# kmaninis/OSVOS-PyTorch

Hardware: NVIDIA H100
Metric: frames/sec at 480x854 fwd-only, batch 1 per GPU (OSVOS.forward -> 5 logit maps) (higher is better)
Workload: dtype bf16x3 (split-bf16 operands, fp32 accumulate)

## Files before the change

### osvos_pytorch_b200/csrc/conv_common.cuh

```cuda
#pragma once
#include <stdlib.h>

#include "common.cuh"
#include "ptx.cuh"

namespace osvos {

constexpr int kTileW = 8;
constexpr int kTileH = 16;
constexpr int kBlockM = 128;
constexpr int kBlockK = 64;
constexpr int kConvThreads = 384;
constexpr int kABytes = kBlockM * kBlockK * 2;

struct ConvParams {
  const float* bias;
  __nv_bfloat16* y_hi;
  __nv_bfloat16* y_lo;
  float* y_f32;
  const __nv_bfloat16* mask_hi;
  __nv_bfloat16* pool_hi;
  __nv_bfloat16* pool_lo;
  float* colsum;
  int n, h, w, cin, cout;
  int tiles_x, tiles_y, n_blocks, total_tiles, k_chunks;
  int flags;
  int ablate;
};

__device__ __forceinline__ void decode_tile(const ConvParams& p, int tile, int& nb, int& tx, int& ty, int& img) {
  nb = tile % p.n_blocks;
  int m = tile / p.n_blocks;
  tx = m % p.tiles_x;
  m /= p.tiles_x;
  ty = m % p.tiles_y;
  img = m / p.tiles_y;
}

__device__ __forceinline__ uint32_t sw128_offset(int row, int chunk) { return row * 128 + ((chunk ^ (row & 7)) << 4); }

__device__ __forceinline__ void split_pack2(float a, float b, uint32_t& hi, uint32_t& lo) {
  asm("cvt.rn.bf16x2.f32 %0, %1, %2;" : "=r"(hi) : "f"(b), "f"(a));
  const float ra = a - __uint_as_float(hi << 16);
  const float rb = b - __uint_as_float(hi & 0xFFFF0000u);
  asm("cvt.rn.bf16x2.f32 %0, %1, %2;" : "=r"(lo) : "f"(rb), "f"(ra));
}

template <int BLOCK_N, bool SPLIT_ACC, bool LEAN = false, bool DET = false>
__device__ __forceinline__ void conv_epilogue(const ConvParams& p, const float* acc, int tile, int wg, int wl, int lane) {
  if (p.ablate & 16) return;
  int nb, tx, ty, img;
  decode_tile(p, tile, nb, tx, ty, img);
  const int lx = lane >> 2;
  const int x = tx * kTileW + lx;
  const int y0 = ty * kTileH + wg * 8 + wl * 2;
  const bool va = (y0 < p.h) && (x < p.w), vb = (y0 + 1 < p.h) && (x < p.w);
  const bool relu = (p.flags & OSVOS_FLAG_RELU) != 0;
  const bool masked = !LEAN && (p.flags & OSVOS_FLAG_RELU_MASK) != 0;
  const bool store_ok = !(p.ablate & 8);
  const size_t pix[2] = {(static_cast<size_t>(img) * p.h + y0) * p.w + x, (static_cast<size_t>(img) * p.h + y0 + 1) * p.w + x};
  const bool valid[2] = {va, vb};
  const int oh = (p.h + 1) >> 1, ow = (p.w + 1) >> 1;
  const bool pool_writer = va && !(lx & 1) && store_ok;
  const size_t opix = (static_cast<size_t>(img) * oh + (y0 >> 1)) * ow + (x >> 1);
#pragma unroll
  for (int j = 0; j < BLOCK_N / 8; ++j) {
    const int c = 8 * j + 2 * (lane & 3);
    const int ch = nb * BLOCK_N + c;
    const float2 b = p.bias ? __ldg(reinterpret_cast<const float2*>(p.bias + ch)) : make_float2(0.f, 0.f);
    float f[2][2];
#pragma unroll
    for (int h = 0; h < 2; ++h) {
#pragma unroll
      for (int e = 0; e < 2; ++e) {
        float v = e ? b.y : b.x;
        v += acc[4 * j + 2 * h + e];
        if (SPLIT_ACC) v += acc[BLOCK_N / 2 + 4 * j + 2 * h + e];
        f[h][e] = relu ? fmaxf(v, 0.f) : v;
      }
    }
#pragma unroll
    for (int h = 0; h < 2; ++h) {
      if (!LEAN && masked && valid[h]) {
        const uint32_t m = __ldg(reinterpret_cast<const unsigned int*>(p.mask_hi + pix[h] * p.cout + ch));
        if (!(bf16_lo_to_float(m) > 0.f)) f[h][0] = 0.f;
        if (!(bf16_hi_to_float(m) > 0.f)) f[h][1] = 0.f;
      }
      if (valid[h] && store_ok) {
        if (!LEAN && p.y_f32) *reinterpret_cast<float2*>(p.y_f32 + pix[h] * p.cout + ch) = make_float2(f[h][0], f[h][1]);
        if (p.y_hi) {
          uint32_t hi, lo;
          split_pack2(f[h][0], f[h][1], hi, lo);
          *reinterpret_cast<uint32_t*>(p.y_hi + pix[h] * p.cout + ch) = hi;
          if (p.y_lo) *reinterpret_cast<uint32_t*>(p.y_lo + pix[h] * p.cout + ch) = lo;
        }
      }
    }
    if (!LEAN && p.colsum) {
      float s0 = (va ? f[0][0] : 0.f) + (vb ? f[1][0] : 0.f);
      float s1 = (va ? f[0][1] : 0.f) + (vb ? f[1][1] : 0.f);
#pragma unroll
      for (int o = 4; o <= 16; o <<= 1) {
        s0 += __shfl_xor_sync(0xffffffffu, s0, o);
        s1 += __shfl_xor_sync(0xffffffffu, s1, o);
      }
      if (lane < 4) {
        if constexpr (DET) {
          const size_t prow = (static_cast<size_t>(tile / p.n_blocks) * 2 + wg) * 4 + wl;
          *reinterpret_cast<float2*>(p.colsum + prow * p.cout + ch) = make_float2(s0, s1);
        } else {
          atomicAdd(p.colsum + ch, s0);
          atomicAdd(p.colsum + ch + 1, s1);
        }
      }
    }
    if (p.pool_hi) {
      float m0 = fmaxf(va ? f[0][0] : -INFINITY, vb ? f[1][0] : -INFINITY);
      float m1 = fmaxf(va ? f[0][1] : -INFINITY, vb ? f[1][1] : -INFINITY);
      m0 = fmaxf(m0, __shfl_xor_sync(0xffffffffu, m0, 4));
      m1 = fmaxf(m1, __shfl_xor_sync(0xffffffffu, m1, 4));
      if (pool_writer) {
        uint32_t hi, lo;
        split_pack2(m0, m1, hi, lo);
        *reinterpret_cast<uint32_t*>(p.pool_hi + opix * p.cout + ch) = hi;
        if (p.pool_lo) *reinterpret_cast<uint32_t*>(p.pool_lo + opix * p.cout + ch) = lo;
      }
    }
  }
}

constexpr int kStageBoxBytes = 64 * 64 * 2;

struct OutMaps {
  CUtensorMap y_hi, y_lo;
};

__device__ __forceinline__ void conv_epilogue_staged(const ConvParams& p, const OutMaps& maps, const float* acc, int tile,
                                                     int half, int wl, int lane, uint8_t* box, int bar_id, bool leader) {
  if (p.ablate & 16) return;
  int nb, tx, ty, img;
  decode_tile(p, tile, nb, tx, ty, img);
  const int lx = lane >> 2;
  const bool relu = (p.flags & OSVOS_FLAG_RELU) != 0;
  const bool store_ok = !(p.ablate & 8);
  const int planes = p.y_lo ? 2 : 1;
  const uint32_t act_row = smem_u32(box) + (wl * 2 * 8 + lx) * 128;
  const uint32_t col = 4 * (lane & 3);
#pragma unroll 1
  for (int plane = 0; plane < planes; ++plane) {
    if (leader) bulk_wait_group_read<0>();
    named_bar_sync(bar_id, 128);
#pragma unroll
    for (int j = 0; j < 8; ++j) {
      const int ch = nb * 64 + 8 * j + 2 * (lane & 3);
      const float2 b = p.bias ? __ldg(reinterpret_cast<const float2*>(p.bias + ch)) : make_float2(0.f, 0.f);
      float f[2][2];
#pragma unroll
      for (int h = 0; h < 2; ++h) {
#pragma unroll
        for (int e = 0; e < 2; ++e) {
          float v = e ? b.y : b.x;
          v += acc[4 * j + 2 * h + e];
          f[h][e] = relu ? fmaxf(v, 0.f) : v;
        }
      }
#pragma unroll
      for (int h = 0; h < 2; ++h) {
        uint32_t hi, lo;
        split_pack2(f[h][0], f[h][1], hi, lo);
        st_shared_u32(act_row + h * 8 * 128 + ((j ^ lx) << 4) + col, plane ? lo : hi);
      }
    }
    fence_proxy_async_smem();
    named_bar_sync(bar_id, 128);
    if (leader && store_ok) {
      tma_store_4d(plane ? &maps.y_lo : &maps.y_hi, box, nb * 64, tx * kTileW, ty * kTileH + half * 8, img);
      bulk_commit_group();
    }
  }
}


static inline void fill_conv_params(ConvParams& p, const osvos_conv3x3_args* a, int block_n) {
  p.bias = a->bias;
  p.y_hi = static_cast<__nv_bfloat16*>(a->y_hi);
  p.y_lo = static_cast<__nv_bfloat16*>(a->y_lo);
  p.y_f32 = a->y_f32;
  p.mask_hi = static_cast<const __nv_bfloat16*>(a->mask_hi);
  p.pool_hi = static_cast<__nv_bfloat16*>(a->pool_hi);
  p.pool_lo = static_cast<__nv_bfloat16*>(a->pool_lo);
  p.colsum = a->colsum;
  p.n = a->n;
  p.h = a->h;
  p.w = a->w;
  p.cin = a->cin;
  p.cout = a->cout;
  p.tiles_x = (a->w + kTileW - 1) / kTileW;
  p.tiles_y = (a->h + kTileH - 1) / kTileH;
  p.n_blocks = a->cout / block_n;
  p.total_tiles = p.tiles_x * p.tiles_y * a->n * p.n_blocks;
  p.k_chunks = a->cin / kBlockK;
  p.flags = a->flags;
  {
    static int ablate = -1;
    if (ablate < 0) {
      const char* e = getenv("OSVOS_ABLATE");
      ablate = e ? atoi(e) : 0;
    }
    p.ablate = ablate;
  }
}

static inline int encode_weight_maps(CUtensorMap* hi, CUtensorMap* lo, const osvos_conv3x3_args* a, int block_n) {
  const size_t plane = static_cast<size_t>(9) * a->cout * a->cin;
  const uint64_t dims[3] = {(uint64_t)a->cin, (uint64_t)a->cout, 9};
  const uint64_t strides[2] = {(uint64_t)a->cin * 2, (uint64_t)a->cout * a->cin * 2};
  const uint32_t box[3] = {kBlockK, (uint32_t)block_n, 1};
  const __nv_bfloat16* wp = static_cast<const __nv_bfloat16*>(a->w_packed);
  int rc = encode_tensor_map(hi, CU_TENSOR_MAP_DATA_TYPE_BFLOAT16, 2, 3, wp, dims, strides, box,
                             CU_TENSOR_MAP_SWIZZLE_128B);
  if (rc) return rc;
  return encode_tensor_map(lo, CU_TENSOR_MAP_DATA_TYPE_BFLOAT16, 2, 3, wp + plane, dims, strides, box,
                           CU_TENSOR_MAP_SWIZZLE_128B);
}

static inline bool outputs_tma_aligned(const osvos_conv3x3_args* a) {
  return ((reinterpret_cast<uintptr_t>(a->y_hi) | reinterpret_cast<uintptr_t>(a->y_lo)) & 15) == 0;
}

static inline int encode_output_maps(OutMaps* m, const osvos_conv3x3_args* a) {
  memset(m, 0, sizeof(*m));
  const uint64_t c = a->cout;
  const uint64_t dims[4] = {c, (uint64_t)a->w, (uint64_t)a->h, (uint64_t)a->n};
  const uint64_t strides[3] = {c * 2, c * 2 * a->w, c * 2 * a->w * a->h};
  const uint32_t box[4] = {64, kTileW, kTileH / 2, 1};
  int rc = encode_tensor_map(&m->y_hi, CU_TENSOR_MAP_DATA_TYPE_BFLOAT16, 2, 4, a->y_hi, dims, strides, box,
                             CU_TENSOR_MAP_SWIZZLE_128B);
  if (rc == OSVOS_OK && a->y_lo)
    rc = encode_tensor_map(&m->y_lo, CU_TENSOR_MAP_DATA_TYPE_BFLOAT16, 2, 4, a->y_lo, dims, strides, box,
                           CU_TENSOR_MAP_SWIZZLE_128B);
  return rc;
}

int conv_first_tc_launch(const float* x, const float* w_oihw, const float* bias, void* y_hi, void* y_lo, int n, int h,
                         int w, int flags, cudaStream_t stream);
int side_conv_dispatch(const osvos_conv3x3_args* a, cudaStream_t stream);
int side_conv_multi_dispatch(const osvos_conv3x3_args* const* args, int count, cudaStream_t stream);

}
```

### osvos_pytorch_b200/csrc/conv_first_tc.cu

```cuda
#include <string.h>

#include "conv_common.cuh"

namespace osvos {

constexpr int kFirstStages = 3;
constexpr int kFirstStageBytes = 2 * kABytes;
constexpr int kFirstBBytes = 2 * 64 * 128;
template <bool STAGED>
constexpr int kFirstSmem = kFirstStages * kFirstStageBytes + kFirstBBytes + (STAGED ? 2 * kStageBoxBytes : 0) + 1024 + 256;

template <int PLANES, bool STAGED>
__global__ void __launch_bounds__(kConvThreads, 1)
conv_first_tc_kernel(const float* __restrict__ x, const float* __restrict__ wgt, const __grid_constant__ OutMaps out,
                     const ConvParams p) {
  extern __shared__ uint8_t smem_raw[];
  uint8_t* smem = reinterpret_cast<uint8_t*>((reinterpret_cast<uintptr_t>(smem_raw) + 1023) & ~uintptr_t(1023));
  uint8_t* smem_b = smem + kFirstStages * kFirstStageBytes;
  uint8_t* smem_stage = smem_b + kFirstBBytes;
  uint64_t* bars = reinterpret_cast<uint64_t*>(smem_stage + (STAGED ? 2 * kStageBoxBytes : 0));
  uint64_t* full_bar = bars;
  uint64_t* empty_bar = bars + kFirstStages;

  const int warp = threadIdx.x >> 5;
  const int lane = threadIdx.x & 31;

  if (threadIdx.x == 0) {
    for (int i = 0; i < kFirstStages; ++i) {
      mbar_init(&full_bar[i], 128);
      mbar_init(&empty_bar[i], 2);
    }
    fence_barrier_init();
  }
  pdl_wait();
  pdl_launch_dependents();
  for (int i = threadIdx.x; i < 64 * 4; i += kConvThreads) {
    const int co = i >> 2, chunk = i & 3;
    uint32_t hi[4], lo[4];
#pragma unroll
    for (int t = 0; t < 4; ++t) {
      const int k0 = chunk * 8 + 2 * t;
      const float v0 = k0 < 27 ? wgt[co * 27 + k0] : 0.f;
      const float v1 = k0 + 1 < 27 ? wgt[co * 27 + k0 + 1] : 0.f;
      __nv_bfloat16 h0, l0, h1, l1;
      split_bf16(v0, h0, l0);
      split_bf16(v1, h1, l1);
      hi[t] = pack_bf16x2(h0, h1);
      lo[t] = pack_bf16x2(l0, l1);
    }
    *reinterpret_cast<uint4*>(smem_b + sw128_offset(co, chunk)) = make_uint4(hi[0], hi[1], hi[2], hi[3]);
    *reinterpret_cast<uint4*>(smem_b + 64 * 128 + sw128_offset(co, chunk)) = make_uint4(lo[0], lo[1], lo[2], lo[3]);
  }
  fence_proxy_async_smem();
  __syncthreads();

  if (warp >= 4) {
    const int wg = (warp - 4) >> 2, wl = warp & 3;
    const bool leader = (threadIdx.x & 127) == 0;
    const uint64_t db_hi = make_smem_desc(smem_b, 16, 1024, kDescSW128);
    const uint64_t db_lo = db_hi + ((64 * 128) >> 4);
    int stage = 0;
    uint32_t phase = 0;
    float acc[32];
    for (int tile = blockIdx.x; tile < p.total_tiles; tile += gridDim.x) {
      mbar_wait(&full_bar[stage], phase);
      const uint64_t da_hi = make_smem_desc(smem + stage * kFirstStageBytes + wg * 64 * 128, 16, 1024, kDescSW128);
      const uint64_t da_lo = da_hi + (kABytes >> 4);
#pragma unroll
      for (int i = 0; i < 32; ++i) acc[i] = 0.f;
      wgmma_fence();
#pragma unroll
      for (int k = 0; k < 2; ++k) {
        if (PLANES == 2) {
          wgmma_bf16<64>(acc, da_lo + 2 * k, db_hi + 2 * k, 1);
          wgmma_bf16<64>(acc, da_hi + 2 * k, db_lo + 2 * k, 1);
        }
        wgmma_bf16<64>(acc, da_hi + 2 * k, db_hi + 2 * k, 1);
      }
      wgmma_commit();
      wgmma_wait<0>();
      wgmma_fence_operands(acc);
      if (leader) mbar_arrive(&empty_bar[stage]);
      if (++stage == kFirstStages) {
        stage = 0;
        phase ^= 1;
      }
      if constexpr (STAGED)
        conv_epilogue_staged(p, out, acc, tile, wg, wl, lane, smem_stage + wg * kStageBoxBytes, 1 + wg, leader);
      else
        conv_epilogue<64, false>(p, acc, tile, wg, wl, lane);
    }
    if (STAGED && leader) bulk_wait_group<0>();
  } else {
    const int row = threadIdx.x;
    const int ly = row / kTileW, lx = row % kTileW;
    int stage = 0;
    uint32_t phase = 0;
    const size_t plane_sz = static_cast<size_t>(p.h) * p.w;
    auto load_tile = [&](int tile, float (&v)[27]) {
      int nb, tx, ty, img;
      decode_tile(p, tile, nb, tx, ty, img);
      const int y = ty * kTileH + ly, xx = tx * kTileW + lx;
#pragma unroll
      for (int ci = 0; ci < 3; ++ci) {
        const float* pl = x + (static_cast<size_t>(img) * 3 + ci) * plane_sz;
#pragma unroll
        for (int r = 0; r < 3; ++r) {
          const int iy = y + r - 1;
#pragma unroll
          for (int s = 0; s < 3; ++s) {
            const int ix = xx + s - 1;
            v[ci * 9 + r * 3 + s] =
                (iy >= 0 && iy < p.h && ix >= 0 && ix < p.w) ? __ldg(pl + static_cast<size_t>(iy) * p.w + ix) : 0.f;
          }
        }
      }
    };
    float vn[27];
    if (static_cast<int>(blockIdx.x) < p.total_tiles) load_tile(blockIdx.x, vn);
    for (int tile = blockIdx.x; tile < p.total_tiles; tile += gridDim.x) {
      float v[32];
#pragma unroll
      for (int k = 0; k < 27; ++k) v[k] = vn[k];
#pragma unroll
      for (int k = 27; k < 32; ++k) v[k] = 0.f;
      if (tile + static_cast<int>(gridDim.x) < p.total_tiles) load_tile(tile + gridDim.x, vn);
      mbar_wait(&empty_bar[stage], phase ^ 1);
      uint8_t* st = smem + stage * kFirstStageBytes;
#pragma unroll
      for (int chunk = 0; chunk < 4; ++chunk) {
        uint32_t hi[4], lo[4];
#pragma unroll
        for (int t = 0; t < 4; ++t) {
          __nv_bfloat16 h0, l0, h1, l1;
          split_bf16(v[chunk * 8 + 2 * t], h0, l0);
          split_bf16(v[chunk * 8 + 2 * t + 1], h1, l1);
          hi[t] = pack_bf16x2(h0, h1);
          lo[t] = pack_bf16x2(l0, l1);
        }
        *reinterpret_cast<uint4*>(st + sw128_offset(row, chunk)) = make_uint4(hi[0], hi[1], hi[2], hi[3]);
        if (PLANES == 2)
          *reinterpret_cast<uint4*>(st + kABytes + sw128_offset(row, chunk)) = make_uint4(lo[0], lo[1], lo[2], lo[3]);
      }
      fence_proxy_async_smem();
      mbar_arrive(&full_bar[stage]);
      if (++stage == kFirstStages) {
        stage = 0;
        phase ^= 1;
      }
    }
  }
}

int conv_first_tc_launch(const float* x, const float* w_oihw, const float* bias, void* y_hi, void* y_lo, int n, int h,
                         int w, int flags, cudaStream_t stream) {
  osvos_conv3x3_args a;
  memset(&a, 0, sizeof(a));
  a.bias = bias;
  a.y_hi = y_hi;
  a.y_lo = (flags & OSVOS_FLAG_FAST) ? nullptr : y_lo;
  a.n = n;
  a.h = h;
  a.w = w;
  a.cin = 64;
  a.cout = 64;
  a.flags = flags;
  ConvParams p;
  fill_conv_params(p, &a, 64);
  const bool fast = (flags & OSVOS_FLAG_FAST) != 0;
  const bool staged = outputs_tma_aligned(&a);
  OutMaps out;
  if (staged) {
    const int rc = encode_output_maps(&out, &a);
    if (rc) return rc;
  } else {
    memset(&out, 0, sizeof(out));
  }
  auto kern = staged ? (fast ? conv_first_tc_kernel<1, true> : conv_first_tc_kernel<2, true>)
                     : (fast ? conv_first_tc_kernel<1, false> : conv_first_tc_kernel<2, false>);
  const int smem = staged ? kFirstSmem<true> : kFirstSmem<false>;
  static uint64_t attr_done[4] = {0, 0, 0, 0};
  OSVOS_CHECK_CUDA(ensure_dynamic_smem(kern, smem, &attr_done[(staged ? 2 : 0) + (fast ? 1 : 0)]));
  const int sms = device_sm_count();
  const int grid = p.total_tiles < sms ? p.total_tiles : sms;
  OSVOS_CHECK_CUDA(launch_pdl(kern, dim3(grid), dim3(kConvThreads), smem, stream, x, w_oihw, out, p));
  return OSVOS_OK;
}

}
```

### osvos_pytorch_b200/csrc/ptx.cuh

```cuda
#pragma once
#include <cuda.h>
#include <cuda_runtime.h>
#include <stdint.h>

#include "wgmma.cuh"

namespace osvos {

#ifndef OSVOS_SPIN_LIMIT
#define OSVOS_SPIN_LIMIT (1u << 26)
#endif

__device__ __forceinline__ uint32_t smem_u32(const void* p) {
  return static_cast<uint32_t>(__cvta_generic_to_shared(p));
}

__device__ __forceinline__ bool elect_one() {
  uint32_t pred = 0;
  asm volatile(
      "{\n\t.reg .pred P;\n\t"
      "elect.sync _|P, 0xffffffff;\n\t"
      "selp.u32 %0, 1, 0, P;\n\t}\n"
      : "=r"(pred));
  return pred != 0;
}

__device__ __forceinline__ void pdl_wait() { asm volatile("griddepcontrol.wait;" ::: "memory"); }
__device__ __forceinline__ void pdl_launch_dependents() { asm volatile("griddepcontrol.launch_dependents;" ::: "memory"); }

__device__ __forceinline__ void mbar_init(uint64_t* bar, uint32_t count) {
  asm volatile("mbarrier.init.shared::cta.b64 [%0], %1;" ::"r"(smem_u32(bar)), "r"(count) : "memory");
}
__device__ __forceinline__ void fence_barrier_init() {
  asm volatile("fence.mbarrier_init.release.cluster;" ::: "memory");
}
__device__ __forceinline__ void fence_proxy_async_smem() {
  asm volatile("fence.proxy.async.shared::cta;" ::: "memory");
}
__device__ __forceinline__ void mbar_arrive_expect_tx(uint64_t* bar, uint32_t bytes) {
  asm volatile("mbarrier.arrive.expect_tx.shared::cta.b64 _, [%0], %1;" ::"r"(smem_u32(bar)), "r"(bytes)
               : "memory");
}
__device__ __forceinline__ void mbar_arrive(uint64_t* bar) {
  asm volatile("mbarrier.arrive.shared::cta.b64 _, [%0];" ::"r"(smem_u32(bar)) : "memory");
}
__device__ __forceinline__ bool mbar_try_wait(uint64_t* bar, uint32_t parity) {
  uint32_t ok;
  asm volatile(
      "{\n\t.reg .pred P;\n\t"
      "mbarrier.try_wait.parity.shared::cta.b64 P, [%1], %2;\n\t"
      "selp.u32 %0, 1, 0, P;\n\t}\n"
      : "=r"(ok)
      : "r"(smem_u32(bar)), "r"(parity)
      : "memory");
  return ok != 0;
}

__device__ __forceinline__ void mbar_wait(uint64_t* bar, uint32_t parity) {
  uint32_t spins = 0;
  while (!mbar_try_wait(bar, parity)) {
    if (++spins > OSVOS_SPIN_LIMIT) __trap();
  }
}

__device__ __forceinline__ void cp_async_8_zfill(void* dst, const void* src, uint32_t src_bytes) {
  asm volatile("cp.async.ca.shared.global [%0], [%1], 8, %2;" ::"r"(smem_u32(dst)), "l"(src), "r"(src_bytes) : "memory");
}
__device__ __forceinline__ void cp_async_mbar_arrive_noinc(uint64_t* bar) {
  asm volatile("cp.async.mbarrier.arrive.noinc.shared::cta.b64 [%0];" ::"r"(smem_u32(bar)) : "memory");
}

__device__ __forceinline__ void tma_prefetch_desc(const CUtensorMap* m) {
  asm volatile("prefetch.tensormap [%0];" ::"l"(reinterpret_cast<uint64_t>(m)) : "memory");
}
__device__ __forceinline__ void tma_load_4d(const CUtensorMap* m, uint64_t* bar, void* dst, int c0, int c1, int c2,
                                            int c3) {
  asm volatile(
      "cp.async.bulk.tensor.4d.shared::cluster.global.mbarrier::complete_tx::bytes"
      " [%0], [%1, {%3, %4, %5, %6}], [%2];"
      ::"r"(smem_u32(dst)), "l"(reinterpret_cast<uint64_t>(m)), "r"(smem_u32(bar)), "r"(c0), "r"(c1), "r"(c2),
      "r"(c3)
      : "memory");
}
__device__ __forceinline__ void tma_load_2d(const CUtensorMap* m, uint64_t* bar, void* dst, int c0, int c1) {
  asm volatile(
      "cp.async.bulk.tensor.2d.shared::cluster.global.mbarrier::complete_tx::bytes"
      " [%0], [%1, {%3, %4}], [%2];"
      ::"r"(smem_u32(dst)), "l"(reinterpret_cast<uint64_t>(m)), "r"(smem_u32(bar)), "r"(c0), "r"(c1)
      : "memory");
}
__device__ __forceinline__ void tma_load_3d(const CUtensorMap* m, uint64_t* bar, void* dst, int c0, int c1, int c2) {
  asm volatile(
      "cp.async.bulk.tensor.3d.shared::cluster.global.mbarrier::complete_tx::bytes"
      " [%0], [%1, {%3, %4, %5}], [%2];"
      ::"r"(smem_u32(dst)), "l"(reinterpret_cast<uint64_t>(m)), "r"(smem_u32(bar)), "r"(c0), "r"(c1), "r"(c2)
      : "memory");
}
__device__ __forceinline__ void st_shared_u32(uint32_t addr, uint32_t v) {
  asm volatile("st.shared.u32 [%0], %1;" ::"r"(addr), "r"(v) : "memory");
}
__device__ __forceinline__ void tma_store_4d(const CUtensorMap* m, const void* src, int c0, int c1, int c2, int c3) {
  asm volatile(
      "cp.async.bulk.tensor.4d.global.shared::cta.bulk_group [%0, {%2, %3, %4, %5}], [%1];"
      ::"l"(reinterpret_cast<uint64_t>(m)), "r"(smem_u32(src)), "r"(c0), "r"(c1), "r"(c2), "r"(c3)
      : "memory");
}
__device__ __forceinline__ void bulk_commit_group() { asm volatile("cp.async.bulk.commit_group;" ::: "memory"); }
template <int N>
__device__ __forceinline__ void bulk_wait_group_read() { asm volatile("cp.async.bulk.wait_group.read %0;" ::"n"(N) : "memory"); }
template <int N>
__device__ __forceinline__ void bulk_wait_group() { asm volatile("cp.async.bulk.wait_group %0;" ::"n"(N) : "memory"); }

constexpr uint64_t kDescSW128 = 1ull << 62;
__host__ __device__ constexpr uint64_t desc_template(uint32_t lbo_bytes, uint32_t sbo_bytes, uint64_t layout) {
  return (static_cast<uint64_t>((lbo_bytes >> 4) & 0x3FFF) << 16) | (static_cast<uint64_t>((sbo_bytes >> 4) & 0x3FFF) << 32) |
         layout;
}
__device__ __forceinline__ uint64_t make_smem_desc(const void* p, uint32_t lbo_bytes, uint32_t sbo_bytes, uint64_t layout) {
  return desc_template(lbo_bytes, sbo_bytes, layout) | static_cast<uint64_t>((smem_u32(p) >> 4) & 0x3FFF);
}

__device__ __forceinline__ void named_bar_sync(int id, int nthreads) {
  asm volatile("bar.sync %0, %1;" ::"r"(id), "r"(nthreads) : "memory");
}
__device__ __forceinline__ void named_bar_arrive(int id, int nthreads) {
  asm volatile("bar.arrive %0, %1;" ::"r"(id), "r"(nthreads) : "memory");
}

template <int N>
__device__ __forceinline__ void setmaxnreg_dec() { asm volatile("setmaxnreg.dec.sync.aligned.u32 %0;" ::"n"(N)); }
template <int N>
__device__ __forceinline__ void setmaxnreg_inc() { asm volatile("setmaxnreg.inc.sync.aligned.u32 %0;" ::"n"(N)); }

struct StageRelease {
  uint64_t* bar_b = nullptr;
  uint64_t* bar_a = nullptr;
  __device__ __forceinline__ void release(bool leader) {
    if (leader) {
      if (bar_b) mbar_arrive(bar_b);
      if (bar_a) mbar_arrive(bar_a);
    }
    bar_b = bar_a = nullptr;
  }
};

}
```

Measured before the change: 659.1.

## Pipeline first-conv input patches via cp.async and per-warp staged TMA epilogue stores

The first-layer producer now loads each tile's 3x18x10 input halo patch into shared memory with a 4-slot cp.async ring, instead of each thread doing 27 guarded global loads with a register prefetch. The staged epilogue is changed from two 128-thread named-barrier rounds per plane to per-warp double-buffered boxes of two rows. These boxes write hi and lo together and issue the TMA stores from lane 0, and each warp waits only for an older slot. This targets global-load latency and epilogue synchronisation, at the cost of more shared memory and smaller TMA store boxes. The output tensor map box changes to 2 rows, which affects every user of encode_output_maps.

```diff
diff --git a/osvos_pytorch_b200/csrc/conv_common.cuh b/osvos_pytorch_b200/csrc/conv_common.cuh
--- a/osvos_pytorch_b200/csrc/conv_common.cuh
+++ b/osvos_pytorch_b200/csrc/conv_common.cuh
@@ -129,54 +129,61 @@
   }
 }
 
-constexpr int kStageBoxBytes = 64 * 64 * 2;
+constexpr int kStageBoxBytes = 16 * 64 * 2;
+constexpr int kStageSlots = 2;
+constexpr int kStageWarpBytes = kStageSlots * 2 * kStageBoxBytes;
 
 struct OutMaps {
   CUtensorMap y_hi, y_lo;
 };
 
 __device__ __forceinline__ void conv_epilogue_staged(const ConvParams& p, const OutMaps& maps, const float* acc, int tile,
-                                                     int half, int wl, int lane, uint8_t* box, int bar_id, bool leader) {
+                                                     int half, int wl, int lane, uint8_t* boxes, int slot) {
   if (p.ablate & 16) return;
   int nb, tx, ty, img;
   decode_tile(p, tile, nb, tx, ty, img);
   const int lx = lane >> 2;
   const bool relu = (p.flags & OSVOS_FLAG_RELU) != 0;
   const bool store_ok = !(p.ablate & 8);
-  const int planes = p.y_lo ? 2 : 1;
-  const uint32_t act_row = smem_u32(box) + (wl * 2 * 8 + lx) * 128;
+  const bool two = p.y_lo != nullptr;
+  uint8_t* box_hi = boxes + slot * 2 * kStageBoxBytes;
+  uint8_t* box_lo = box_hi + kStageBoxBytes;
+  const uint32_t act_row = smem_u32(box_hi) + lx * 128;
   const uint32_t col = 4 * (lane & 3);
-#pragma unroll 1
-  for (int plane = 0; plane < planes; ++plane) {
-    if (leader) bulk_wait_group_read<0>();
-    named_bar_sync(bar_id, 128);
-#pragma unroll
-    for (int j = 0; j < 8; ++j) {
-      const int ch = nb * 64 + 8 * j + 2 * (lane & 3);
-      const float2 b = p.bias ? __ldg(reinterpret_cast<const float2*>(p.bias + ch)) : make_float2(0.f, 0.f);
-      float f[2][2];
-#pragma unroll
-      for (int h = 0; h < 2; ++h) {
-#pragma unroll
-        for (int e = 0; e < 2; ++e) {
-          float v = e ? b.y : b.x;
-          v += acc[4 * j + 2 * h + e];
-          f[h][e] = relu ? fmaxf(v, 0.f) : v;
-        }
-      }
-#pragma unroll
-      for (int h = 0; h < 2; ++h) {
-        uint32_t hi, lo;
-        split_pack2(f[h][0], f[h][1], hi, lo);
-        st_shared_u32(act_row + h * 8 * 128 + ((j ^ lx) << 4) + col, plane ? lo : hi);
-      }
-    }
-    fence_proxy_async_smem();
-    named_bar_sync(bar_id, 128);
-    if (leader && store_ok) {
-      tma_store_4d(plane ? &maps.y_lo : &maps.y_hi, box, nb * 64, tx * kTileW, ty * kTileH + half * 8, img);
-      bulk_commit_group();
-    }
+  if (lane == 0) bulk_wait_group_read<kStageSlots - 1>();
+  __syncwarp();
+#pragma unroll
+  for (int j = 0; j < 8; ++j) {
+    const int ch = nb * 64 + 8 * j + 2 * (lane & 3);
+    const float2 b = p.bias ? __ldg(reinterpret_cast<const float2*>(p.bias + ch)) : make_float2(0.f, 0.f);
+    float f[2][2];
+#pragma unroll
+    for (int h = 0; h < 2; ++h) {
+#pragma unroll
+      for (int e = 0; e < 2; ++e) {
+        float v = e ? b.y : b.x;
+        v += acc[4 * j + 2 * h + e];
+        f[h][e] = relu ? fmaxf(v, 0.f) : v;
+      }
+    }
+#pragma unroll
+    for (int h = 0; h < 2; ++h) {
+      uint32_t hi, lo;
+      split_pack2(f[h][0], f[h][1], hi, lo);
+      const uint32_t at = act_row + h * 8 * 128 + ((j ^ lx) << 4) + col;
+      st_shared_u32(at, hi);
+      if (two) st_shared_u32(at + kStageBoxBytes, lo);
+    }
+  }
+  fence_proxy_async_smem();
+  __syncwarp();
+  if (lane == 0) {
+    if (store_ok) {
+      const int y = ty * kTileH + half * 8 + wl * 2;
+      tma_store_4d(&maps.y_hi, box_hi, nb * 64, tx * kTileW, y, img);
+      if (two) tma_store_4d(&maps.y_lo, box_lo, nb * 64, tx * kTileW, y, img);
+    }
+    bulk_commit_group();
   }
 }
 
@@ -233,7 +240,7 @@
   const uint64_t c = a->cout;
   const uint64_t dims[4] = {c, (uint64_t)a->w, (uint64_t)a->h, (uint64_t)a->n};
   const uint64_t strides[3] = {c * 2, c * 2 * a->w, c * 2 * a->w * a->h};
-  const uint32_t box[4] = {64, kTileW, kTileH / 2, 1};
+  const uint32_t box[4] = {64, kTileW, 2, 1};
   int rc = encode_tensor_map(&m->y_hi, CU_TENSOR_MAP_DATA_TYPE_BFLOAT16, 2, 4, a->y_hi, dims, strides, box,
                              CU_TENSOR_MAP_SWIZZLE_128B);
   if (rc == OSVOS_OK && a->y_lo)
diff --git a/osvos_pytorch_b200/csrc/conv_first_tc.cu b/osvos_pytorch_b200/csrc/conv_first_tc.cu
--- a/osvos_pytorch_b200/csrc/conv_first_tc.cu
+++ b/osvos_pytorch_b200/csrc/conv_first_tc.cu
@@ -7,8 +7,12 @@
 constexpr int kFirstStages = 3;
 constexpr int kFirstStageBytes = 2 * kABytes;
 constexpr int kFirstBBytes = 2 * 64 * 128;
+constexpr int kPatchW = kTileW + 2, kPatchH = kTileH + 2;
+constexpr int kPatchFloats = 3 * kPatchH * kPatchW;
+constexpr int kFirstPatchSlots = 4;
 template <bool STAGED>
-constexpr int kFirstSmem = kFirstStages * kFirstStageBytes + kFirstBBytes + (STAGED ? 2 * kStageBoxBytes : 0) + 1024 + 256;
+constexpr int kFirstSmem = kFirstStages * kFirstStageBytes + kFirstBBytes + (STAGED ? 8 * kStageWarpBytes : 0) +
+                           kFirstPatchSlots * kPatchFloats * 4 + 1024 + 256;
 
 template <int PLANES, bool STAGED>
 __global__ void __launch_bounds__(kConvThreads, 1)
@@ -18,7 +22,8 @@
   uint8_t* smem = reinterpret_cast<uint8_t*>((reinterpret_cast<uintptr_t>(smem_raw) + 1023) & ~uintptr_t(1023));
   uint8_t* smem_b = smem + kFirstStages * kFirstStageBytes;
   uint8_t* smem_stage = smem_b + kFirstBBytes;
-  uint64_t* bars = reinterpret_cast<uint64_t*>(smem_stage + (STAGED ? 2 * kStageBoxBytes : 0));
+  float* patches = reinterpret_cast<float*>(smem_stage + (STAGED ? 8 * kStageWarpBytes : 0));
+  uint64_t* bars = reinterpret_cast<uint64_t*>(patches + kFirstPatchSlots * kPatchFloats);
   uint64_t* full_bar = bars;
   uint64_t* empty_bar = bars + kFirstStages;
 
@@ -59,7 +64,8 @@
     const bool leader = (threadIdx.x & 127) == 0;
     const uint64_t db_hi = make_smem_desc(smem_b, 16, 1024, kDescSW128);
     const uint64_t db_lo = db_hi + ((64 * 128) >> 4);
-    int stage = 0;
+    uint8_t* boxes = smem_stage + (warp - 4) * kStageWarpBytes;
+    int stage = 0, slot = 0;
     uint32_t phase = 0;
     float acc[32];
     for (int tile = blockIdx.x; tile < p.total_tiles; tile += gridDim.x) {
@@ -85,59 +91,78 @@
         stage = 0;
         phase ^= 1;
       }
-      if constexpr (STAGED)
-        conv_epilogue_staged(p, out, acc, tile, wg, wl, lane, smem_stage + wg * kStageBoxBytes, 1 + wg, leader);
-      else
+      if constexpr (STAGED) {
+        conv_epilogue_staged(p, out, acc, tile, wg, wl, lane, boxes, slot);
+        if (++slot == kStageSlots) slot = 0;
+      } else {
         conv_epilogue<64, false>(p, acc, tile, wg, wl, lane);
-    }
-    if (STAGED && leader) bulk_wait_group<0>();
+      }
+    }
+    if (STAGED && lane == 0) bulk_wait_group<0>();
   } else {
     const int row = threadIdx.x;
     const int ly = row / kTileW, lx = row % kTileW;
-    int stage = 0;
-    uint32_t phase = 0;
     const size_t plane_sz = static_cast<size_t>(p.h) * p.w;
-    auto load_tile = [&](int tile, float (&v)[27]) {
+    constexpr int kLoads = (kPatchFloats + 127) / 128;
+    int prow[kLoads], pcol[kLoads];
+    long long poff[kLoads];
+#pragma unroll
+    for (int k = 0; k < kLoads; ++k) {
+      const int e = threadIdx.x + 128 * k;
+      const int ci = e / (kPatchH * kPatchW), rc = e % (kPatchH * kPatchW);
+      prow[k] = rc / kPatchW - 1;
+      pcol[k] = rc % kPatchW - 1;
+      poff[k] = static_cast<long long>(ci) * static_cast<long long>(plane_sz) + static_cast<long long>(prow[k]) * p.w + pcol[k];
+    }
+    auto load_patch = [&](int tile, int slot) {
       int nb, tx, ty, img;
       decode_tile(p, tile, nb, tx, ty, img);
-      const int y = ty * kTileH + ly, xx = tx * kTileW + lx;
-#pragma unroll
-      for (int ci = 0; ci < 3; ++ci) {
-        const float* pl = x + (static_cast<size_t>(img) * 3 + ci) * plane_sz;
-#pragma unroll
-        for (int r = 0; r < 3; ++r) {
-          const int iy = y + r - 1;
-#pragma unroll
-          for (int s = 0; s < 3; ++s) {
-            const int ix = xx + s - 1;
-            v[ci * 9 + r * 3 + s] =
-                (iy >= 0 && iy < p.h && ix >= 0 && ix < p.w) ? __ldg(pl + static_cast<size_t>(iy) * p.w + ix) : 0.f;
-          }
+      const int y0 = ty * kTileH, x0 = tx * kTileW;
+      const float* base = x + static_cast<size_t>(img) * 3 * plane_sz + static_cast<size_t>(y0) * p.w + x0;
+      float* dst = patches + slot * kPatchFloats + threadIdx.x;
+#pragma unroll
+      for (int k = 0; k < kLoads; ++k) {
+        if (threadIdx.x + 128 * k < kPatchFloats) {
+          const bool in = static_cast<unsigned>(y0 + prow[k]) < static_cast<unsigned>(p.h) &&
+                          static_cast<unsigned>(x0 + pcol[k]) < static_cast<unsigned>(p.w);
+          cp_async_4_zfill(dst + 128 * k, in ? base + poff[k] : x, in ? 4u : 0u);
         }
       }
     };
-    float vn[27];
-    if (static_cast<int>(blockIdx.x) < p.total_tiles) load_tile(blockIdx.x, vn);
+    int next = blockIdx.x, fill = 0;
+    for (int i = 0; i < kFirstPatchSlots - 1; ++i) {
+      if (next < p.total_tiles) load_patch(next, fill);
+      cp_async_commit_group();
+      next += gridDim.x;
+      ++fill;
+    }
+    int stage = 0, slot = 0;
+    uint32_t phase = 0;
     for (int tile = blockIdx.x; tile < p.total_tiles; tile += gridDim.x) {
+      cp_async_wait_group<kFirstPatchSlots - 2>();
+      named_bar_sync(1, 128);
+      if (next < p.total_tiles) load_patch(next, fill);
+      cp_async_commit_group();
+      next += gridDim.x;
+      if (++fill == kFirstPatchSlots) fill = 0;
+      const float* pt = patches + slot * kPatchFloats + ly * kPatchW + lx;
+      if (++slot == kFirstPatchSlots) slot = 0;
       float v[32];
 #pragma unroll
-      for (int k = 0; k < 27; ++k) v[k] = vn[k];
+      for (int ci = 0; ci < 3; ++ci)
+#pragma unroll
+        for (int r = 0; r < 3; ++r)
+#pragma unroll
+          for (int s = 0; s < 3; ++s) v[ci * 9 + r * 3 + s] = pt[(ci * kPatchH + r) * kPatchW + s];
 #pragma unroll
       for (int k = 27; k < 32; ++k) v[k] = 0.f;
-      if (tile + static_cast<int>(gridDim.x) < p.total_tiles) load_tile(tile + gridDim.x, vn);
       mbar_wait(&empty_bar[stage], phase ^ 1);
       uint8_t* st = smem + stage * kFirstStageBytes;
 #pragma unroll
       for (int chunk = 0; chunk < 4; ++chunk) {
         uint32_t hi[4], lo[4];
 #pragma unroll
-        for (int t = 0; t < 4; ++t) {
-          __nv_bfloat16 h0, l0, h1, l1;
-          split_bf16(v[chunk * 8 + 2 * t], h0, l0);
-          split_bf16(v[chunk * 8 + 2 * t + 1], h1, l1);
-          hi[t] = pack_bf16x2(h0, h1);
-          lo[t] = pack_bf16x2(l0, l1);
-        }
+        for (int t = 0; t < 4; ++t) split_pack2(v[chunk * 8 + 2 * t], v[chunk * 8 + 2 * t + 1], hi[t], lo[t]);
         *reinterpret_cast<uint4*>(st + sw128_offset(row, chunk)) = make_uint4(hi[0], hi[1], hi[2], hi[3]);
         if (PLANES == 2)
           *reinterpret_cast<uint4*>(st + kABytes + sw128_offset(row, chunk)) = make_uint4(lo[0], lo[1], lo[2], lo[3]);
diff --git a/osvos_pytorch_b200/csrc/ptx.cuh b/osvos_pytorch_b200/csrc/ptx.cuh
--- a/osvos_pytorch_b200/csrc/ptx.cuh
+++ b/osvos_pytorch_b200/csrc/ptx.cuh
@@ -66,6 +66,12 @@
 __device__ __forceinline__ void cp_async_8_zfill(void* dst, const void* src, uint32_t src_bytes) {
   asm volatile("cp.async.ca.shared.global [%0], [%1], 8, %2;" ::"r"(smem_u32(dst)), "l"(src), "r"(src_bytes) : "memory");
 }
+__device__ __forceinline__ void cp_async_4_zfill(void* dst, const void* src, uint32_t src_bytes) {
+  asm volatile("cp.async.ca.shared.global [%0], [%1], 4, %2;" ::"r"(smem_u32(dst)), "l"(src), "r"(src_bytes) : "memory");
+}
+__device__ __forceinline__ void cp_async_commit_group() { asm volatile("cp.async.commit_group;" ::: "memory"); }
+template <int N>
+__device__ __forceinline__ void cp_async_wait_group() { asm volatile("cp.async.wait_group %0;" ::"n"(N) : "memory"); }
 __device__ __forceinline__ void cp_async_mbar_arrive_noinc(uint64_t* bar) {
   asm volatile("cp.async.mbarrier.arrive.noinc.shared::cta.b64 [%0];" ::"r"(smem_u32(bar)) : "memory");
 }
```

New measurement: 661.6 (median of 6 runs). About the same (+0.4%).
